# facebookresearch/robust-dynrf

Measured on AMD Instinct MI355X. Metric: training rays/sec (Nvidia Balloon1, configs/Nvidia.txt, static+dynamic TensorVMSplit), higher is better.
Workload: dtype f32; 1 GPU; BASELINE.json configs[1]: Nvidia Balloon1, configs/Nvidia.txt, 4096 rays/iter/GPU, 1xMI355X per rank, static+dynamic TensorVMSplit; one step = 5 dynamic + 5 static forward passes, scene-flow MLP, induced flow/disparity, per-frame depth loss, distortion loss, compositor, factor regularisers, full backward, Adam; config=nvidia, stage=stage0, samples_per_ray=115, global_batch=4096, rays_per_gpu=4096, parallelism=ray-sharded dp1, ranks=1, dead_work=executed (work the reference also computes although nothing consumes it)

## Files before the change

include/rodynrf.h:

```cpp
#ifndef RODYNRF_H
#define RODYNRF_H
#include <stddef.h>
#include <stdint.h>

#ifdef __cplusplus
extern "C" {
#endif

#define RDRF_ABI_VERSION 6

typedef void* rdrf_stream_t;

enum { RDRF_RAY_NDC = 0, RDRF_RAY_CONTRACT = 1, RDRF_RAY_OTHER = 2 };
enum { RDRF_ACT_RELU = 0, RDRF_ACT_SOFTPLUS = 1 };
enum { RDRF_HEAD_MLP_FEA = 0, RDRF_HEAD_MLP_FEA_TIMEEMBEDDING = 1 };
enum { RDRF_SCATTER_RAY = 0, RDRF_SCATTER_SORTED = 1, RDRF_SCATTER_AUTO = 2, RDRF_SCATTER_SORTED_PLAIN = 3 };

typedef struct {
  float* plane[3];
  float* line[3];
  int C[3];
  int H[3], W[3];
  int L[3];
  int sH[3], sW[3];
// ... 321 lines not shown
                      float* y, void* ws, size_t ws_bytes, rdrf_stream_t stream);

#define RDRF_ST_F32 0
#define RDRF_ST_F32_T 1
#define RDRF_ST_B3 2
#define RDRF_ST_B3_T 3
#define RDRF_ST_B3_PAIR_T 4
#define RDRF_ST_B3S 5
#define RDRF_ST_B3S_T 6
int rdrf_selftest_layer(int form, const float* x, const float* w, int M, int K, int OUT, float* y, void* ws, size_t ws_bytes,
                        rdrf_stream_t stream);

#define RDRF_DW_DENSITY 0
#define RDRF_DW_STATIC_FEA 1
#define RDRF_DW_STATIC_TE 2
#define RDRF_DW_DYN_APP 3
#define RDRF_DW_DYN 4
#define RDRF_DW_SCENE_FLOW 5
#define RDRF_DW_FEAT_STATIC 6
#define RDRF_DW_FEAT_DYN 7
#define RDRF_DW_LIVE_D 1
#define RDRF_DW_LIVE_B 2
#define RDRF_DW_SMALL_IN_KERNEL 4
int rdrf_selftest_dw(int plan, int flags, const float* A, size_t A_floats, const float* B, size_t B_floats, int ntiles,
                     const int* count, const void* grads, rdrf_stream_t stream);
int rdrf_selftest_dw_describe(int plan, int flags, int* out, int cap);
int rdrf_selftest_sf_geometry(int ntiles, int* grid, int* waves);

void rdrf_prof_reset(void);
int rdrf_prof_enable(int on);
int rdrf_prof_get(const char* kernel, double* total_ms, int* launches);

#ifdef __cplusplus
}
#endif
#endif
```

robust-dynrf_amd/_lib.py:

```python
import ctypes as C
import os

import torch

_HERE = os.path.dirname(os.path.abspath(__file__))
DETERMINISTIC = os.environ.get("RDRF_DETERMINISTIC", "0") == "1"
LIB_PATH = os.environ.get("RDRF_LIB", os.path.join(_HERE, "librodynrf_det.so" if DETERMINISTIC else "librodynrf.so"))

ABI_VERSION = 6

RAY_TYPES = {"ndc": 0, "contract": 1}
ACTS = {"relu": 0, "softplus": 1}
HEADS = {"MLP_Fea": 0, "MLP_Fea_TimeEmbedding": 1}
SAVE_NO_APP = 1

fp = C.POINTER(C.c_float)


class RdrfVM(C.Structure):
    _fields_ = [("plane", C.c_void_p * 3), ("line", C.c_void_p * 3), ("C", C.c_int * 3),
                ("H", C.c_int * 3), ("W", C.c_int * 3), ("L", C.c_int * 3),
                ("sH", C.c_int * 3), ("sW", C.c_int * 3)]


# ... 102 lines not shown
    lib.rdrf_render_chunks_maps_fwd.argtypes = [C.c_void_p, C.c_void_p, C.c_void_p, C.c_void_p, C.c_void_p, C.c_void_p,
                                                C.c_int, C.c_int, C.c_int, C.c_float, C.c_float, C.POINTER(RenderMapsC),
                                                C.c_void_p, C.c_size_t, C.c_void_p, C.c_void_p, C.c_int]
    lib.rdrf_render_motion_workspace_bytes.restype = C.c_size_t
    lib.rdrf_render_motion_workspace_bytes.argtypes = [C.c_int, C.c_int]
    lib.rdrf_render_motion_fwd.argtypes = [C.c_void_p, C.c_void_p, C.c_void_p, C.c_void_p, C.c_void_p, C.c_void_p, C.c_int,
                                           C.c_int, C.c_float, C.c_float, C.c_int, C.POINTER(RenderMapsC),
                                           C.POINTER(MotionCamsC), C.POINTER(MotionMapsC), C.c_void_p, C.c_size_t, C.c_void_p]
    lib.rdrf_flow_to_image_workspace_bytes.restype = C.c_size_t
    lib.rdrf_flow_to_image_workspace_bytes.argtypes = [C.c_int, C.c_int]
    lib.rdrf_flow_to_image.argtypes = [C.c_void_p, C.c_int, C.c_int, C.c_void_p, C.c_void_p, C.c_size_t, C.c_void_p]
    lib.rdrf_camera_rays.argtypes = [C.c_void_p, C.c_void_p, C.c_int, C.c_int, C.c_int, C.c_int, C.c_float, C.c_int64,
                                     C.c_int, C.c_void_p, C.c_void_p]
    lib.rdrf_ssim_workspace_bytes.restype = C.c_size_t
    lib.rdrf_ssim_workspace_bytes.argtypes = [C.c_int, C.c_int, C.c_int]
    lib.rdrf_ssim.argtypes = [C.c_void_p, C.c_void_p, C.c_int, C.c_int, C.c_int, C.c_float, C.c_void_p, C.c_void_p,
                              C.c_void_p, C.c_size_t, C.c_void_p]
    lib.rdrf_gather_batch.argtypes = [C.POINTER(SceneTablesC), C.c_void_p, C.c_void_p, C.c_int, C.POINTER(BatchC), C.c_void_p]
    lib.rdrf_selftest_layer.argtypes = [C.c_int, C.c_void_p, C.c_void_p, C.c_int, C.c_int, C.c_int, C.c_void_p, C.c_void_p,
                                        C.c_size_t, C.c_void_p]
    lib.rdrf_selftest_dw.argtypes = [C.c_int, C.c_int, C.c_void_p, C.c_size_t, C.c_void_p, C.c_size_t, C.c_int, C.c_void_p,
                                     C.c_void_p, C.c_void_p]
    lib.rdrf_selftest_dw_describe.argtypes = [C.c_int, C.c_int, C.POINTER(C.c_int), C.c_int]
    lib.rdrf_prof_get.argtypes = [C.c_char_p, C.POINTER(C.c_double), C.POINTER(C.c_int)]
    lib.rdrf_det_bind.argtypes = [C.c_int, C.c_void_p, C.c_size_t, C.c_void_p, C.c_void_p]
    lib.rdrf_det_finish.argtypes = [C.c_int, C.c_void_p]
    if DETERMINISTIC and not lib.rdrf_deterministic():
        raise ImportError(f"RDRF_DETERMINISTIC=1 but {LIB_PATH} is the product build")
    return lib


lib = _load()

SYMBOLS = [
    "rdrf_abi_version", "rdrf_last_error", "rdrf_workspace_bytes", "rdrf_forward_workspace_bytes", "rdrf_saved_bytes", "rdrf_saved_bytes_ex", "rdrf_saved_row_bytes",
    "rdrf_generate_rays",
    "rdrf_generate_rays_bwd", "rdrf_generate_rays_uv", "rdrf_generate_rays_uv_bwd", "rdrf_sample_ndc", "rdrf_sample_contract", "rdrf_sample_bwd",
    "rdrf_static_fwd", "rdrf_static_fwd_ex", "rdrf_static_bwd", "rdrf_dynamic_fwd", "rdrf_dynamic_fwd_ex", "rdrf_dynamic_bwd",
    "rdrf_features_saved_bytes", "rdrf_features_workspace_bytes", "rdrf_features_bwd_workspace_bytes",
    "rdrf_static_features_fwd", "rdrf_static_features_bwd", "rdrf_dynamic_features_fwd",
    "rdrf_dynamic_features_bwd",
    "rdrf_scene_flow_fwd", "rdrf_scene_flow_bwd", "rdrf_composite_fwd", "rdrf_composite_bwd",
    "rdrf_induce_flow_fwd", "rdrf_induce_flow_bwd", "rdrf_rows_scatter_add", "rdrf_distloss_fwd", "rdrf_distloss_bwd",
    "rdrf_tv_fwd", "rdrf_tv_bwd", "rdrf_tv_grad", "rdrf_adam_step", "rdrf_upsample_bilinear", "rdrf_dense_l1_fwd",
    "rdrf_dense_l1_bwd", "rdrf_pack_floats", "rdrf_static_pack", "rdrf_dynamic_pack", "rdrf_loss_terms_workspace_floats", "rdrf_loss_terms_fwd", "rdrf_loss_terms_bwd",
    "rdrf_loss_terms_stats", "rdrf_loss_terms_finish", "rdrf_deterministic", "rdrf_det_bind", "rdrf_det_finish",
    "rdrf_render_fused_fwd", "rdrf_render_sequence_fwd",
    "rdrf_frame_depth_loss_workspace_bytes", "rdrf_frame_depth_loss_fwd", "rdrf_frame_depth_loss_bwd",
    "rdrf_render_workspace_bytes", "rdrf_render_fwd", "rdrf_render_chunks_workspace_bytes", "rdrf_render_chunks_fwd",
    "rdrf_render_maps_fwd", "rdrf_render_chunks_maps_fwd", "rdrf_camera_rays", "rdrf_ssim_workspace_bytes", "rdrf_ssim",
    "rdrf_render_motion_workspace_bytes", "rdrf_render_motion_fwd", "rdrf_flow_to_image_workspace_bytes", "rdrf_flow_to_image",
    "rdrf_gather_batch",
    "rdrf_set_scatter_mode", "rdrf_selftest_mlp", "rdrf_selftest_layer", "rdrf_selftest_dw", "rdrf_selftest_dw_describe",
    "rdrf_selftest_sf_geometry",
    "rdrf_prof_reset",
    "rdrf_prof_enable", "rdrf_prof_get",
]


SELFTEST_FORMS = {"F32": 0, "F32_T": 1, "B3": 2, "B3_T": 3, "B3_PAIR_T": 4, "B3S": 5, "B3S_T": 6}

DW_PLANS = {"DENSITY": 0, "STATIC_FEA": 1, "STATIC_TE": 2, "DYN_APP": 3, "DYN": 4, "SCENE_FLOW": 5, "FEAT_STATIC": 6, "FEAT_DYN": 7}
DW_LIVE_D, DW_LIVE_B, DW_SMALL_IN_KERNEL = 1, 2, 4

SCATTER_MODES = {"ray": 0, "sorted": 1, "auto": 2, "sorted_plain": 3}


def set_scatter_mode(mode):
    check(lib.rdrf_set_scatter_mode(SCATTER_MODES[mode]), "rdrf_set_scatter_mode")


class RdrfTensor4(C.Structure):
    _fields_ = [("x", C.c_void_p), ("g", C.c_void_p), ("C", C.c_int), ("H", C.c_int), ("W", C.c_int),
                ("sC", C.c_longlong), ("sH", C.c_longlong), ("sW", C.c_longlong)]


TV_MAX = 16


class RdrfLossTerm(C.Structure):
    _fields_ = [("x", C.c_void_p), ("y", C.c_void_p), ("w", C.c_void_p), ("gx", C.c_void_p), ("gy", C.c_void_p),
                ("rows", C.c_longlong), ("cols", C.c_int), ("kind", C.c_int), ("norm", C.c_int),
                ("ysign", C.c_float), ("coef", C.c_float), ("coef_dev", C.c_void_p)]


MAX_LOSS_TERMS = 32
# ... 66 lines not shown
```

robust-dynrf_amd/csrc/rdrf_bwd.hip:

```cpp
#ifdef RDRF_GROWS_TEMPORAL
#define RDRF_SAVE_TEMPORAL
#endif
#include "rdrf_bwd_dev.hpp"
#include "rdrf_bwd_host.hpp"

RDRF_DET_UNIT(bwd)

RDRF_D void x0_bwd(const float (&X0)[32], const float (&dX0)[32], int h, float& d0, float& d1,
                   float& d2) {
#pragma unroll
  for (int o = 0; o < 8; ++o) {
    if (o == 0 && h == 0) {
      d0 += dX0[0]; d1 += dX0[1]; d2 += dX0[2];
    } else {
      const int k = 2 * o + h - 1;
#pragma unroll
      for (int p = 0; p < 2; ++p) {
        const int j = 2 * k + p;
        const int d = j / 10, f = j - d * 10;
        const float sv = X0[o * 4 + 2 * p], cv = X0[o * 4 + 2 * p + 1];
        const float dq = ldexpf(dX0[o * 4 + 2 * p] * cv - dX0[o * 4 + 2 * p + 1] * sv, f);
        d0 += d == 0 ? dq : 0.f; d1 += d == 1 ? dq : 0.f; d2 += d == 2 ? dq : 0.f;
      }
    }
  }
}

RDRF_D float act_grad(float f, int act, float shift) {
  return act == RDRF_ACT_RELU ? (f > 0.0f ? 1.0f : 0.0f) : sigmoidf_(f + shift);
}

template <int KK, int NO>
// ... 1159 lines not shown
      const int rr = e >> 6, hh = (e >> 5) & 1, c = e & 31;
      const int col = seg_imap(layer == 0 ? SEG_SF_X : SEG_IDENT, 32 * k + c, in_dim);
      const int orow = bo * 32 + (rr & 3) + 8 * (rr >> 2) + 4 * hh;
      if (col >= 0) grad_add(G.w[layer] + (size_t)orow * in_dim + col, red[p * 1024 + e]);
    }
  }
#pragma unroll
  for (int a = 0; a < sfd::NDZ; ++a) {
    const int layer = 2 - (a >> 1), orow = (a & 1) * 32 + (int)threadIdx.x;
    if (threadIdx.x < 32)
      grad_add(G.b[layer] + orow, red[sfd::NPROD * 1024 + a * 64 + threadIdx.x] + red[sfd::NPROD * 1024 + a * 64 + 32 + threadIdx.x]);
  }
  for (int e = threadIdx.x; e < 12 * 32 + 6; e += blockDim.x) {
    const int a = e < 12 * 32 ? e >> 5 : 12 + (e - 12 * 32), c = e < 12 * 32 ? e & 31 : 0;
    const float* r = red + sfd::NPROD * 1024 + (sfd::NDZ + a) * 64 + c;
    if (a < 12) grad_add(G.w[3] + (a >> 1) * 64 + (a & 1) * 32 + c, r[0] + r[32]);
    else grad_add(G.b[3] + (a - 12), r[0] + r[32]);
  }
}
void scene_flow_fused_geometry(long tiles, int* grid, int* waves) {
  const long blocks = (tiles + SFD_WAVES - 1) / SFD_WAVES;
  *grid = (int)(blocks < 1 ? 1 : (blocks > 256 ? 256 : blocks));
  *waves = SFD_WAVES;
}

void fill_static_w(StaticW& w, const RdrfStaticParams* P);
void fill_dyn_w(DynW& w, const RdrfDynamicParams* P);

static void dyn_pack_jobs_bwd(PackJobs& J, const RdrfDynamicParams* P) {
  using namespace pkb;
  J.n = 0;
  const int kh = REG_K1H, kw = REG_K1W, k3 = REG_K3, sf = REG_SF;
  pack_add(J, P->l5w, 64, 3, 64, SEG_IDENT, 1, 3, 32, kw + K1W_W5);
#ifdef RDRF_HEADS_BWD_F32
  const int wm = 2;
#else
  const int wm = 8;
#endif
  pack_add(J, P->l4w, 64, 64, 64, SEG_IDENT, wm, 2, 32, kw + K1W_W4T);
  pack_add(J, P->l3w, 93, 64, 93, SEG_WARP3_X0, wm, 2, 32, kw + K1W_W3T_X0);
  pack_add(J, P->l3w, 93, 64, 93, SEG_WARP3_T, wm, 1, 32, kw + K1W_W3T_T);
  pack_add(J, P->dw2, 64, 1, 64, SEG_IDENT, 1, 1, 32, kh + K1H_DEN2);
  pack_add(J, P->bw2, 64, 1, 64, SEG_IDENT, 1, 1, 32, kh + K1H_BLE2);
#ifdef RDRF_HEADS_BWD_F32
  const int hm = 2;
#else
// ... 97 lines not shown
  b.dxn = dynamic ? c.take<float>(ns * 3) : nullptr;
  b.dtout = dynamic ? c.take<float>((size_t)N * 32) : nullptr;
  b.gf = dynamic ? nullptr : c.take<float>(t1 * 32);
  b.dfs = nullptr;
  b.dfa = nullptr;
  b.gsig = b.dtp = nullptr;
  if (dynamic) {
    b.dfs = c.take<float>(ns * DFS_FLOATS);
    b.dfa = c.take<float>(ns * DFA_FLOATS);
    b.keys_in = c.take<unsigned>(3 * ns);
    b.keys_out = c.take<unsigned>(3 * ns);
    b.order = c.take<unsigned>(3 * ns);
    b.counts = c.take<int>(64);
    b.sort_tmp_bytes = rdrf_sort_temp_bytes((unsigned)(3 * ns), 32);
    b.sort_tmp = c.take<char>(b.sort_tmp_bytes);
    b.gsig = c.take<float>(ns);
    b.dtp = c.take<float>(t3 * 64);
  }
  RDRF_CHECK(c.ok(), -3, "backward workspace too small: need %zu have %zu", c.off, ws_bytes);
  return 0;
}

void add_density_phase_dw(DwJobs& D, const float* grows1, const float* act1, const RdrfDynamicParams* G, int T1, bool live_d,
                          bool live_b, bool small_in_kernel) {
  dw_add(D, grows1, sv::K1G_ROWS, sv::K1G_DZ3, 2, 64, 0, act1, sv::K1_ROWS, 93, 93, G->l3w, G->l3b, nullptr, T1);
  dw_blk(D, sv::K1_X0, SEG_WARP3_X0, 0);
  dw_blk(D, sv::K1_X0 + 32, SEG_WARP3_X0, 32);
  dw_blk(D, sv::K1_T, SEG_WARP3_T, 0);
  dw_add(D, grows1, sv::K1G_ROWS, sv::K1G_DZ4, 2, 64, 0, act1, sv::K1_ROWS, 64, 64, G->l4w, G->l4b, nullptr, T1);
  dw_blk(D, sv::K1_H3, SEG_IDENT, 0);
  dw_blk(D, sv::K1_H3 + 32, SEG_IDENT, 32);
  if (!small_in_kernel) {
  dw_add(D, grows1, sv::K1G_ROWS, sv::K1G_SM, 1, 3, 0, act1, sv::K1_ROWS, 64, 64, G->l5w, G->l5b, nullptr, T1);
  dw_blk(D, sv::K1_H4, SEG_IDENT, 0);
  dw_blk(D, sv::K1_H4 + 32, SEG_IDENT, 32);
  if (live_d) {
    dw_add(D, grows1, sv::K1G_ROWS, sv::K1G_SM, 1, 1, 3, act1, sv::K1_ROWS, 64, 64, G->dw2, G->db2, nullptr, T1);
    dw_blk(D, sv::K1_HD, SEG_IDENT, 0);
    dw_blk(D, sv::K1_HD + 32, SEG_IDENT, 32);
  }
  if (live_b) {
    dw_add(D, grows1, sv::K1G_ROWS, sv::K1G_SM, 1, 1, 4, act1, sv::K1_ROWS, 64, 64, G->bw2, G->bb2, nullptr, T1);
    dw_blk(D, sv::K1_HB, SEG_IDENT, 0);
    dw_blk(D, sv::K1_HB + 32, SEG_IDENT, 32);
  }
  }
  for (int head = 0; head < 2; ++head) {
    if (!(head ? live_b : live_d)) continue;
    dw_add(D, grows1, sv::K1G_ROWS, head ? sv::K1G_DZB : sv::K1G_DZD, 2, 64, 0, act1, sv::K1_ROWS, 152, 152,
           head ? G->bw1 : G->dw1, head ? G->bb1 : G->db1, nullptr, T1);
    const int f0 = head ? sv::K1_FB : sv::K1_FD;
    dw_blk(D, f0, SEG_IDENT72, 0);
    dw_blk(D, f0 + 32, SEG_IDENT72, 32);
    dw_blk(D, f0 + 64, SEG_IDENT72, 64);
    dw_blk(D, sv::K1_X0, SEG_DEN1_X0, 0);
    dw_blk(D, sv::K1_X0 + 32, SEG_DEN1_X0, 32);
    dw_blk(D, sv::K1_X1, SEG_DEN1_X1, 0);
  }
}
void add_static_app_dw(DwJobs& D, const float* grows3, const float* act3, const RdrfStaticParams* G, bool fea, const int* cnt,
                       int ntiles) {
  const int in1 = fea ? 138 : 135;
  dw_add(D, grows3, sv::K3G_ROWS, sv::K3G_DZV, 1, 3, 0, act3, sv::S3_ROWS, 128,
         fea ? 128 : 131, G->w3, G->b3, cnt, ntiles);
  for (int i = 0; i < 4; ++i) dw_blk(D, sv::S3_H2 + 32 * i, SEG_IDENT, 32 * i);
  if (!fea) dw_blk(D, sv::S3_VD, SEG_VIEW3, 0);
  dw_add(D, grows3, sv::K3G_ROWS, sv::K3G_DF, 1, 27, 0, act3, sv::S3_ROWS, 72, 72, G->basis,
         nullptr, cnt, ntiles);
  for (int i = 0; i < 3; ++i) dw_blk(D, sv::S3_G + 32 * i, SEG_IDENT, 32 * i);
  dw_add(D, grows3, sv::K3G_ROWS, sv::K3G_DZ2, 4, 128, 0, act3, sv::S3_ROWS, 128, 128, G->w2,
         G->b2, cnt, ntiles);
  for (int i = 0; i < 4; ++i) dw_blk(D, sv::S3_H1 + 32 * i, SEG_IDENT, 32 * i);
  dw_add(D, grows3, sv::K3G_ROWS, sv::K3G_DZ1, 4, 128, 0, act3, sv::S3_ROWS, in1, in1, G->w1,
         G->b1, cnt, ntiles);
  dw_blk(D, sv::S3_F, fea ? SEG_STAT1_F_FEA : SEG_STAT1_F_TE, 0);
  for (int i = 0; i < 4; ++i) dw_blk(D, sv::S3_P + 32 * i, fea ? SEG_STAT1_P_FEA : SEG_STAT1_P_TE, 32 * i);
}
void add_dyn_app_dw(DwJobs& D, const float* grows3, const float* act3, const RdrfDynamicParams* G, const int* cnt, int ntiles) {
  dw_add(D, grows3, sv::K3G_ROWS, sv::K3G_DZV, 1, 3, 0, act3, sv::K3_ROWS, 128, 131, G->rwv,
         G->rbv, cnt, ntiles);
  for (int i = 0; i < 4; ++i) dw_blk(D, sv::K3_H2 + 32 * i, SEG_IDENT, 32 * i);
// ... 195 lines not shown
    } else RDRF_LAUNCH("dyn_heads_bwd", (k_dyn_density_bwd<0, false>), dim3(g.grid), dim3(g.block), stream, a, w, gw);
    if (smode != 0) {
      const int set_mask = ((g_sigma != nullptr || g_weight != nullptr) ? 1 : 0) | (g_blending != nullptr ? 2 : 0);
      if (set_mask != 0) {
        rdrf_prof_begin("scatter_dyn_density", stream);
        rc = scatter_dyn_density_sorted(a, b, P, G, set_mask, stream);
        rdrf_prof_end("scatter_dyn_density", stream);
        if (rc) return rc;
      }
    } else {
      const bool has_d = g_sigma != nullptr || g_weight != nullptr, has_b = g_blending != nullptr;
      if (has_d || has_b) {
        ScatterArgs sa;
        fill_scatter_common(sa, a);
        sa.nsets = 0;
        if (has_d) { sa.vm[sa.nsets] = P->density; sa.gvm[sa.nsets] = G->density; sa.row0[sa.nsets] = sv::K1G_DFD; ++sa.nsets; }
        if (has_b) { sa.vm[sa.nsets] = P->blending; sa.gvm[sa.nsets] = G->blending; sa.row0[sa.nsets] = sv::K1G_DFB; ++sa.nsets; }
        sa.rows = b.grows1; sa.stride = sv::K1G_ROWS; sa.flat = flat ? 1 : 0;
        sa.xw = a.sp.xw;
        sa.dxw = b.dxw; sa.dxw_accumulate = 1;
        { int rc_ = launch_scatter("scatter_dyn_density", SCATTER_4_1_9, sa, (long)t1, stream); if (rc_) return rc_; }
      }
    }
    if (flat) RDRF_LAUNCH("dyn_warp_bwd", (k_dyn_density_bwd<1, false, true>), dim3(g.grid), dim3(g.block), stream, a, w, gw);
    else RDRF_LAUNCH("dyn_warp_bwd", (k_dyn_density_bwd<1, false>), dim3(g.grid), dim3(g.block), stream, a, w, gw);
    RDRF_LAUNCH("time_branch_bwd", k_time_branch_bwd, dim3((N + TB_RPB - 1) / TB_RPB), dim3(128), stream, ts, w,
                N, b.dtout, flat ? (const float*)b.dtp : nullptr, S, G->l1w, G->l1b, G->l2w, G->l2b);
    const bool small_in_kernel = a.small_dw != 0;
    add_density_phase_dw(D, b.grows1, a.sp.act1, G, (int)t1, g_sigma != nullptr || g_weight != nullptr, g_blending != nullptr,
                         small_in_kernel);
  }
  rc = dw_launch(D, stream, "dw_dyn");
  return rc;
}

struct FeatWs {
  float *pk, *grows3, *grows1, *dxw, *dxn, *dtout, *gpad, *xpad;
  uint8_t* valid;
};
static int carve_feat_bwd(FeatWs& b, void* ws, size_t ws_bytes, int M, int dynamic) {
  WsCarver c(ws, ws_bytes);
  const size_t t = ((size_t)M + 31) / 32, mp = t * 32;
  b.pk = c.take<float>(PACK_AREA_FLOATS);
  b.grows3 = c.take<float>(t * sv::K3G_ROWS * 32);
  b.grows1 = dynamic ? c.take<float>(t * sv::K1G_ROWS * 32) : nullptr;
  b.dxw = dynamic ? c.take<float>(mp * 3) : nullptr;
  b.dxn = dynamic ? c.take<float>(mp * 3) : nullptr;
  b.dtout = dynamic ? c.take<float>(mp * 32) : nullptr;
  b.gpad = dynamic ? nullptr : c.take<float>(mp);
  b.xpad = dynamic ? nullptr : c.take<float>(mp * 3);
  b.valid = c.take<uint8_t>(mp);
  RDRF_CHECK(c.ok(), -3, "features backward: workspace too small: need %zu have %zu", c.off, ws_bytes);
  return 0;
// ... 184 lines not shown
  const int T = (int)tiles;
  DwJobs D;
  D.n = 0;
  add_scene_flow_dw(D, grows, act, G, T);
  return dw_launch(D, stream, "dw_sf");
}

void dyn_pack_jobs_fwd(PackJobs& J, const RdrfDynamicParams* P);
void static_pack_jobs_fwd(PackJobs& J, const RdrfStaticParams* P, int head);
extern "C" size_t rdrf_pack_floats(void) { return PACK_AREA_FLOATS; }
extern "C" int rdrf_static_pack(const RdrfStaticParams* P, int static_head, int backward, float* image,
                                rdrf_stream_t stream_) {
  RDRF_CHECK(P && image && (((uintptr_t)image) & 15) == 0, -1, "static_pack: bad arguments");
  PackJobs J;
  if (backward) static_pack_jobs_bwd(J, P, static_head); else static_pack_jobs_fwd(J, P, static_head);
  return pack_launch(J, image, (hipStream_t)stream_);
}
extern "C" int rdrf_dynamic_pack(const RdrfDynamicParams* P, int backward, float* image, rdrf_stream_t stream_) {
  RDRF_CHECK(P && image && (((uintptr_t)image) & 15) == 0, -1, "dynamic_pack: bad arguments");
  PackJobs J;
  if (backward) dyn_pack_jobs_bwd(J, P); else dyn_pack_jobs_fwd(J, P);
  return pack_launch(J, image, (hipStream_t)stream_);
}
```

robust-dynrf_amd/csrc/rdrf_bwd_host.hpp:

```cpp
#pragma once
#include "rdrf_host.hpp"

struct BwdArgs;

struct BwdWs {
  float* dfs;
  float* dfa;
  unsigned *keys_in, *keys_out, *order;
  int* counts;
  void* sort_tmp;
  size_t sort_tmp_bytes;
  float* pk;
  float* gf;
  float* grows1;
  float* grows3;
  float* dxw;
  float* dxn;
  float* dtout;
  float* gsig;
  float* dtp;
};

struct ScatterArgs {
  RdrfVM vm[2], gvm[2];
// ... 33 lines not shown
  const float* A;
  int A_stride, A_row0, nbo, out_dim, out_row0;
  const float* B;
  int B_stride;
  int nblk;
  int blk_row0[8], blk_seg[8], blk_e0[8];
  int in_dim, ld;
  float* dW;
  float* db;
  const int* count;
  int ntiles;
};
#define RDRF_MAX_DW_JOBS 12
struct DwJobs {
  DwJob j[RDRF_MAX_DW_JOBS];
  int n;
};
void dw_add(DwJobs& D, const float* A, int A_stride, int A_row0, int nbo, int out_dim, int out_row0, const float* B,
            int B_stride, int in_dim, int ld, float* dW, float* db, const int* count, int ntiles);
void dw_blk(DwJobs& D, int row0, int seg, int e0);
int dw_launch(DwJobs& D, hipStream_t stream, const char* name);

void add_density_phase_dw(DwJobs& D, const float* grows1, const float* act1, const RdrfDynamicParams* G, int T1,
                          bool live_d = true, bool live_b = true, bool small_in_kernel = false);
void add_static_app_dw(DwJobs& D, const float* grows3, const float* act3, const RdrfStaticParams* G, bool fea, const int* cnt,
                       int ntiles);
void add_dyn_app_dw(DwJobs& D, const float* grows3, const float* act3, const RdrfDynamicParams* G, const int* cnt, int ntiles);
void add_scene_flow_dw(DwJobs& D, const float* grows, const float* act, const RdrfDynamicParams* G, int T);
void add_feat_static_dw(DwJobs& D, const float* grows3, const float* act3, const RdrfStaticParams* G, int Np);
void add_feat_dyn_app_dw(DwJobs& D, const float* grows3, const float* act3, const RdrfDynamicParams* G, int Np);
void scene_flow_fused_geometry(long tiles, int* grid, int* waves);
```

robust-dynrf_amd/csrc/rdrf_selftest.hip:

```cpp
#include "rdrf_bwd_host.hpp"

namespace {

template <int KK>
RDRF_D void st_load(float (&in)[KK], const float* __restrict__ x, int row, int M, int ld, int c0, int h) {
#pragma unroll
  for (int kk = 0; kk < KK; ++kk) in[kk] = row < M ? x[(size_t)row * ld + c0 + elem_of(kk, h)] : 0.f;
}
template <int NBO>
RDRF_D void st_store(const f32x16 (&acc)[NBO], float* __restrict__ y, int row, int M, int ld, int c0, int h) {
  if (row < M)
#pragma unroll
    for (int nb = 0; nb < NBO; ++nb)
#pragma unroll
      for (int r = 0; r < 16; ++r) y[(size_t)row * ld + c0 + nb * 32 + elem_of(r, h)] = acc[nb][r];
}

template <int NBO, int KK>
__global__ __launch_bounds__(64) void k_st_f32(const float* __restrict__ x, const float* __restrict__ pkw, int M,
                                               float* __restrict__ y) {
  constexpr int IMG = NBO * KK * 64;
  __shared__ __attribute__((aligned(16))) float lds[IMG];
  lds_fill(lds, pkw, IMG);
  const int lane = threadIdx.x & 63, h = lane >> 5, row = blockIdx.x * 32 + (lane & 31);
// ... 169 lines not shown
      if (OUT == 32 && nbi == 3) ST_RUN(img + nbi * kk * 32, (k_st_b3s_t<3, 16>));
      if (OUT == 128 && nbi == 4) ST_RUN(img + nbi * kk * 32, (k_st_b3s_t<4, 64>));
      if (OUT == 128 && nbi == 3) ST_RUN(img + nbi * kk * 32, (k_st_b3s_t<3, 64>));
      if (OUT == 128 && nbi == 5) ST_RUN(img + nbi * kk * 32, (k_st_b3s_t<5, 64>));
      break;
    }
  }
  rdrf_set_error("selftest_layer: form %d is not instantiated for K = %d, OUT = %d", form, K, OUT);
  return -1;
}

namespace {

struct DwPlanInfo {
  int dynamic;
  int region[RDRF_MAX_DW_JOBS];
  int nregions;
};

int dw_plan_jobs(int plan, int flags, const float* A, const float* B, size_t ntiles, const int* count, const void* G, DwJobs& D,
                 DwPlanInfo& I) {
  const RdrfStaticParams* Gs = (const RdrfStaticParams*)G;
  const RdrfDynamicParams* Gd = (const RdrfDynamicParams*)G;
  const bool live_d = (flags & RDRF_DW_LIVE_D) != 0, live_b = (flags & RDRF_DW_LIVE_B) != 0, small = (flags & RDRF_DW_SMALL_IN_KERNEL) != 0;
  const int T = (int)ntiles, Tc = count ? 0 : T;
  D.n = 0;
  I.dynamic = 1;
  int n0 = -1;
  const float *A1 = nullptr, *B1 = nullptr;
  auto second = [&]() {
    n0 = D.n;
    A1 = A + ntiles * (size_t)D.j[0].A_stride * 32;
    B1 = B + ntiles * (size_t)D.j[0].B_stride * 32;
  };
  switch (plan) {
    case RDRF_DW_DENSITY: add_density_phase_dw(D, A, B, Gd, T, live_d, live_b, small); break;
    case RDRF_DW_STATIC_FEA: I.dynamic = 0; add_static_app_dw(D, A, B, Gs, true, count, Tc); break;
    case RDRF_DW_STATIC_TE: I.dynamic = 0; add_static_app_dw(D, A, B, Gs, false, count, Tc); break;
    case RDRF_DW_DYN_APP: add_dyn_app_dw(D, A, B, Gd, count, Tc); break;
    case RDRF_DW_DYN:
      add_dyn_app_dw(D, A, B, Gd, count, Tc);
      second();
      add_density_phase_dw(D, A1, B1, Gd, T, live_d, live_b, small);
      break;
    case RDRF_DW_SCENE_FLOW: add_scene_flow_dw(D, A, B, Gd, T); break;
    case RDRF_DW_FEAT_STATIC: I.dynamic = 0; add_feat_static_dw(D, A, B, Gs, T); break;
    case RDRF_DW_FEAT_DYN:
      add_feat_dyn_app_dw(D, A, B, Gd, T);
      second();
      add_density_phase_dw(D, A1, B1, Gd, T, live_d, live_b);
      break;
    default: rdrf_set_error("selftest_dw: unknown plan %d", plan); return -1;
  }
  I.nregions = n0 < 0 ? 1 : 2;
  for (int j = 0; j < D.n; ++j) I.region[j] = (n0 >= 0 && j >= n0) ? 1 : 0;
  return 0;
}

}

extern "C" int rdrf_selftest_dw(int plan, int flags, const float* A, size_t A_floats, const float* B, size_t B_floats, int ntiles,
                                const int* count, const void* grads, rdrf_stream_t stream_) {
  hipStream_t stream = (hipStream_t)stream_;
  DwJobs D;
  DwPlanInfo I;
  RDRF_CHECK(plan >= RDRF_DW_DENSITY && plan <= RDRF_DW_FEAT_DYN, -1, "selftest_dw: unknown plan %d", plan);
// ... 43 lines not shown
    while (j < D.n && I.region[j] != g) ++j;
    out[n++] = D.j[j].A_stride; out[n++] = D.j[j].B_stride; out[n++] = D.j[j].count != nullptr ? 1 : 0;
  }
  for (int j = 0; j < D.n; ++j) {
    const DwJob& J = D.j[j];
    out[n++] = I.region[j]; out[n++] = J.A_row0; out[n++] = J.nbo; out[n++] = J.out_dim; out[n++] = J.out_row0;
    out[n++] = J.in_dim; out[n++] = J.ld;
    out[n++] = (int)((uintptr_t)J.dW - 8);
    out[n++] = J.db != nullptr ? (int)((uintptr_t)J.db - 8) : -1;
    out[n++] = J.nblk;
    for (int k = 0; k < J.nblk; ++k) {
      out[n++] = J.blk_row0[k];
      for (int li = 0; li < 32; ++li) out[n++] = seg_imap(J.blk_seg[k], J.blk_e0[k] + li, J.in_dim);
    }
  }
  return n;
}

extern "C" int rdrf_selftest_sf_geometry(int ntiles, int* grid, int* waves) {
  RDRF_CHECK(ntiles >= 0 && grid && waves, -1, "selftest_sf_geometry: bad arguments");
  scene_flow_fused_geometry(ntiles, grid, waves);
  return 0;
}
```

Baseline: 460,200 rays/s.

## Fuse warp-MLP backward with its weight-gradient reductions into one kernel

Adds a fused warp-branch backward kernel that computes the layer 3/4/5 activation gradients and also accumulates the weight and bias gradients in registers through MFMA outer products. Partial sums are reduced across waves in LDS and then added to global memory. The kernel is enabled by default on the flat, small-dw path, and the separate dw jobs for l3/l4 are dropped when it runs. The goal is to avoid writing dz3/dz4 rows to global memory and launching dw GEMM jobs for them. The cost is higher register and LDS pressure and a grid capped at 256 blocks, which can limit occupancy.

```diff
diff --git a/include/rodynrf.h b/include/rodynrf.h
--- a/include/rodynrf.h
+++ b/include/rodynrf.h
@@ -367,10 +367,17 @@
 #define RDRF_DW_LIVE_D 1
 #define RDRF_DW_LIVE_B 2
 #define RDRF_DW_SMALL_IN_KERNEL 4
+#define RDRF_DW_WARP_IN_KERNEL 8
 int rdrf_selftest_dw(int plan, int flags, const float* A, size_t A_floats, const float* B, size_t B_floats, int ntiles,
                      const int* count, const void* grads, rdrf_stream_t stream);
 int rdrf_selftest_dw_describe(int plan, int flags, int* out, int cap);
 int rdrf_selftest_sf_geometry(int ntiles, int* grid, int* waves);
+int rdrf_selftest_warp_geometry(int ntiles, int* grid, int* waves);
+size_t rdrf_selftest_warp_bwd_workspace_bytes(int N, int S);
+int rdrf_selftest_warp_bwd(const RdrfDynamicParams* P, const RdrfFieldCfg* cfg, int N, int S, const float* act1,
+                           size_t act1_floats, float* grows1, size_t grows1_floats, float* dxw, float* dxn,
+                           const float* g_xyz_prime, const RdrfDynamicParams* grads, float* g_xyz, float* dtout, float* dtp,
+                           void* ws, size_t ws_bytes, rdrf_stream_t stream);
 
 void rdrf_prof_reset(void);
 int rdrf_prof_enable(int on);
diff --git a/robust-dynrf_amd/_lib.py b/robust-dynrf_amd/_lib.py
--- a/robust-dynrf_amd/_lib.py
+++ b/robust-dynrf_amd/_lib.py
@@ -148,6 +148,12 @@
     lib.rdrf_selftest_dw.argtypes = [C.c_int, C.c_int, C.c_void_p, C.c_size_t, C.c_void_p, C.c_size_t, C.c_int, C.c_void_p,
                                      C.c_void_p, C.c_void_p]
     lib.rdrf_selftest_dw_describe.argtypes = [C.c_int, C.c_int, C.POINTER(C.c_int), C.c_int]
+    lib.rdrf_selftest_warp_geometry.argtypes = [C.c_int, C.POINTER(C.c_int), C.POINTER(C.c_int)]
+    lib.rdrf_selftest_warp_bwd_workspace_bytes.restype = C.c_size_t
+    lib.rdrf_selftest_warp_bwd_workspace_bytes.argtypes = [C.c_int, C.c_int]
+    lib.rdrf_selftest_warp_bwd.argtypes = [C.c_void_p, C.c_void_p, C.c_int, C.c_int, C.c_void_p, C.c_size_t, C.c_void_p, C.c_size_t,
+                                           C.c_void_p, C.c_void_p, C.c_void_p, C.c_void_p, C.c_void_p, C.c_void_p, C.c_void_p,
+                                           C.c_void_p, C.c_size_t, C.c_void_p]
     lib.rdrf_prof_get.argtypes = [C.c_char_p, C.POINTER(C.c_double), C.POINTER(C.c_int)]
     lib.rdrf_det_bind.argtypes = [C.c_int, C.c_void_p, C.c_size_t, C.c_void_p, C.c_void_p]
     lib.rdrf_det_finish.argtypes = [C.c_int, C.c_void_p]
@@ -178,7 +184,7 @@
     "rdrf_render_motion_workspace_bytes", "rdrf_render_motion_fwd", "rdrf_flow_to_image_workspace_bytes", "rdrf_flow_to_image",
     "rdrf_gather_batch",
     "rdrf_set_scatter_mode", "rdrf_selftest_mlp", "rdrf_selftest_layer", "rdrf_selftest_dw", "rdrf_selftest_dw_describe",
-    "rdrf_selftest_sf_geometry",
+    "rdrf_selftest_sf_geometry", "rdrf_selftest_warp_geometry", "rdrf_selftest_warp_bwd_workspace_bytes", "rdrf_selftest_warp_bwd",
     "rdrf_prof_reset",
     "rdrf_prof_enable", "rdrf_prof_get",
 ]
@@ -187,7 +193,7 @@
 SELFTEST_FORMS = {"F32": 0, "F32_T": 1, "B3": 2, "B3_T": 3, "B3_PAIR_T": 4, "B3S": 5, "B3S_T": 6}
 
 DW_PLANS = {"DENSITY": 0, "STATIC_FEA": 1, "STATIC_TE": 2, "DYN_APP": 3, "DYN": 4, "SCENE_FLOW": 5, "FEAT_STATIC": 6, "FEAT_DYN": 7}
-DW_LIVE_D, DW_LIVE_B, DW_SMALL_IN_KERNEL = 1, 2, 4
+DW_LIVE_D, DW_LIVE_B, DW_SMALL_IN_KERNEL, DW_WARP_IN_KERNEL = 1, 2, 4, 8
 
 SCATTER_MODES = {"ray": 0, "sorted": 1, "auto": 2, "sorted_plain": 3}
 
diff --git a/robust-dynrf_amd/csrc/rdrf_bwd.hip b/robust-dynrf_amd/csrc/rdrf_bwd.hip
--- a/robust-dynrf_amd/csrc/rdrf_bwd.hip
+++ b/robust-dynrf_amd/csrc/rdrf_bwd.hip
@@ -8,6 +8,7 @@
 
 RDRF_D void x0_bwd(const float (&X0)[32], const float (&dX0)[32], int h, float& d0, float& d1,
                    float& d2) {
+#pragma clang fp contract(off)
 #pragma unroll
   for (int o = 0; o < 8; ++o) {
     if (o == 0 && h == 0) {
@@ -1213,6 +1214,264 @@
   const long blocks = (tiles + SFD_WAVES - 1) / SFD_WAVES;
   *grid = (int)(blocks < 1 ? 1 : (blocks > 256 ? 256 : blocks));
   *waves = SFD_WAVES;
+}
+
+namespace wpd {
+constexpr int WAVES = SFD_WAVES;
+constexpr int ST_SIZE = 64 * 32;
+constexpr int NPROD = 10, NDZ = 4, NSM = 6;
+constexpr int LDS = pkb::K1W_SIZE + WAVES * ST_SIZE;
+constexpr int RED = NPROD * 1024 + (NDZ + NSM) * 64;
+static_assert(pkb::K1W_SIZE % 4 == 0 && RED <= LDS && LDS * 4 <= 160 * 1024, "the cross-wave sum reuses the kernel's LDS");
+}
+struct WarpGrads {
+  float *l3w, *l3b, *l4w, *l4b;
+};
+RDRF_D void x0_bwd_flat(const float (&X0)[32], const float (&dX0)[32], int h, float& d0, float& d1, float& d2) {
+#pragma clang fp contract(off)
+  d0 += h == 0 ? dX0[0] : 0.f; d1 += h == 0 ? dX0[1] : 0.f; d2 += h == 0 ? dX0[2] : 0.f;
+#pragma unroll
+  for (int o = 0; o < 8; ++o) {
+    const int k = 2 * o + h - 1;
+#pragma unroll
+    for (int p = 0; p < 2; ++p) {
+      const int j = 2 * k + p;
+      const int d = j >= 0 ? j / 10 : -1, f = j >= 0 ? j - d * 10 : 0;
+      const float sv = X0[o * 4 + 2 * p], cv = X0[o * 4 + 2 * p + 1];
+      const float dq = ldexpf(dX0[o * 4 + 2 * p] * cv - dX0[o * 4 + 2 * p + 1] * sv, f);
+      d0 += d == 0 ? dq : 0.f; d1 += d == 1 ? dq : 0.f; d2 += d == 2 ? dq : 0.f;
+    }
+  }
+}
+
+template <bool GX>
+__global__ __launch_bounds__(64 * wpd::WAVES) void k_dyn_warp_bwd_dw(BwdArgs a, DynG gw, WarpGrads G) {
+  __shared__ __attribute__((aligned(16))) float lds[wpd::LDS];
+  const int lane = threadIdx.x & 63, h = lane >> 5, s = lane & 31;
+  const int wave = __builtin_amdgcn_readfirstlane(threadIdx.x >> 6), nwaves = blockDim.x >> 6;
+  float* st = lds + pkb::K1W_SIZE + wave * wpd::ST_SIZE;
+  lds_fill(lds, a.pk + pkb::REG_K1W, pkb::K1W_SIZE);
+  const int total = a.N * a.S;
+  const int ntiles = (total + 31) >> 5;
+  const SfdPos pos = sfd_lane_pos(s, h);
+  f32x16 accW[wpd::NPROD];
+  float bsum[wpd::NDZ];
+  float sw[3] = {0.f, 0.f, 0.f}, sb[3] = {0.f, 0.f, 0.f};
+  acc_zero<wpd::NPROD>(accW);
+#pragma unroll
+  for (int i = 0; i < wpd::NDZ; ++i) bsum[i] = 0.f;
+  for (int n = blockIdx.x * nwaves + wave; n < ntiles; n += gridDim.x * nwaves) {
+    const bool act = n * 32 + s < total;
+    const int idx = act ? n * 32 + s : 0;
+    const float* svb = a.sp.act1 + (size_t)n * sv::K1_ROWS * 32;
+    float* gb = a.grows1 + (size_t)n * sv::K1G_ROWS * 32;
+    float dw0 = act ? a.dxw_app[(size_t)idx * 3 + 0] : 0.f, dw1 = act ? a.dxw_app[(size_t)idx * 3 + 1] : 0.f,
+          dw2 = act ? a.dxw_app[(size_t)idx * 3 + 2] : 0.f;
+    float dn0 = act ? a.dxn_app[(size_t)idx * 3 + 0] : 0.f, dn1 = act ? a.dxn_app[(size_t)idx * 3 + 1] : 0.f,
+          dn2 = act ? a.dxn_app[(size_t)idx * 3 + 2] : 0.f;
+    float dd0 = dw0 * a.box.inv[0], dd1 = dw1 * a.box.inv[1], dd2 = dw2 * a.box.inv[2];
+    float gp0 = 0.f, gp1 = 0.f, gp2 = 0.f;
+    if (act && a.g_xyz_prime) {
+      gp0 = a.g_xyz_prime[(size_t)idx * 3 + 0]; gp1 = a.g_xyz_prime[(size_t)idx * 3 + 1];
+      gp2 = a.g_xyz_prime[(size_t)idx * 3 + 2];
+    }
+    dd0 += gp0; dd1 += gp1; dd2 += gp2;
+    if (!act) { dd0 = dd1 = dd2 = 0.f; }
+    if (h == 0) {
+      gb[(size_t)(sv::K1G_SM + 0) * 32 + s] = dd0; gb[(size_t)(sv::K1G_SM + 1) * 32 + s] = dd1;
+      gb[(size_t)(sv::K1G_SM + 2) * 32 + s] = dd2;
+    }
+    float dz4[32];
+    {
+      float H4[32];
+      load_rows<32>(svb, sv::K1_H4, H4, s, h);
+      const float* w5 = lds + pkb::K1W_W5 + h * 32;
+#pragma unroll
+      for (int q = 0; q < 8; ++q) {
+        const f32x4 wa = *reinterpret_cast<const f32x4*>(w5 + 4 * q);
+        const f32x4 wb = *reinterpret_cast<const f32x4*>(w5 + 64 + 4 * q);
+        const f32x4 wc = *reinterpret_cast<const f32x4*>(w5 + 128 + 4 * q);
+#pragma unroll
+        for (int c = 0; c < 4; ++c) {
+          const float d = wa[c] * dd0 + wb[c] * dd1 + wc[c] * dd2;
+          dz4[4 * q + c] = H4[4 * q + c] > 0.f ? d : 0.f;
+        }
+      }
+      sb[0] += dd0; sb[1] += dd1; sb[2] += dd2;
+#pragma unroll 1
+      for (int o = 0; o < 3; ++o) {
+        const float dd = o == 0 ? dd0 : (o == 1 ? dd1 : dd2);
+        float pw[32];
+#pragma unroll
+        for (int kk = 0; kk < 32; ++kk) pw[kk] = dd * H4[kk];
+        const float r = reduce_scatter32(pw, s);
+        sw[0] += o == 0 ? r : 0.f; sw[1] += o == 1 ? r : 0.f; sw[2] += o == 2 ? r : 0.f;
+      }
+    }
+    f32x4 b0[4], b1[4], b2[4];
+    sfd_wave_sync();
+    sfd_stage(st, dz4, pos);
+    sfd_wave_sync();
+    sfd_load(b0, svb, sv::K1_H3 + s, h);
+    sfd_load(b1, svb, sv::K1_H3 + 32 + s, h);
+    float dz3[32];
+    {
+      f32x16 acc[2];
+      acc_zero<2>(acc);
+#ifdef RDRF_HEADS_BWD_F32
+      mfma_seg<2, 32>(acc, dz4, lds + pkb::K1W_W4T, lane);
+#else
+      mfma_seg_b3<2, 32>(acc, dz4, lds + pkb::K1W_W4T, lane);
+#endif
+      float H3[32];
+      load_rows<32>(svb, sv::K1_H3, H3, s, h);
+#pragma unroll
+      for (int bo = 0; bo < 2; ++bo) {
+        f32x4 av[4];
+        sfd_read(av, st, bo, pos);
+        bsum[bo] += sfd_sum(av);
+        sfd_prod(accW[2 * bo], av, b0);
+        sfd_prod(accW[2 * bo + 1], av, b1);
+        __builtin_amdgcn_sched_barrier(0);
+      }
+#pragma unroll
+      for (int kk = 0; kk < 32; ++kk) dz3[kk] = H3[kk] > 0.f ? acc[kk >> 4][kk & 15] : 0.f;
+    }
+    sfd_wave_sync();
+    sfd_stage(st, dz3, pos);
+    sfd_wave_sync();
+    sfd_load(b0, svb, sv::K1_X0 + s, h);
+    sfd_load(b1, svb, sv::K1_X0 + 32 + s, h);
+    sfd_load(b2, svb, sv::K1_T + s, h);
+    f32x16 accX[2];
+    {
+      float dXh[32];
+      load_rows<32>(gb, sv::K1G_DX0, dXh, s, h);
+#pragma unroll
+      for (int kk = 0; kk < 32; ++kk) accX[kk >> 4][kk & 15] = dXh[kk];
+    }
+    f32x16 accT[1];
+    acc_zero<1>(accT);
+#ifdef RDRF_HEADS_BWD_F32
+    mfma_seg<2, 32>(accX, dz3, lds + pkb::K1W_W3T_X0, lane);
+    mfma_seg<1, 32>(accT, dz3, lds + pkb::K1W_W3T_T, lane);
+#else
+    mfma_seg_b3_pair<2, 1, 32>(accX, accT, dz3, lds + pkb::K1W_W3T_X0, lds + pkb::K1W_W3T_T, lane);
+#endif
+#pragma unroll
+    for (int bo = 0; bo < 2; ++bo) {
+      f32x4 av[4];
+      sfd_read(av, st, bo, pos);
+      bsum[2 + bo] += sfd_sum(av);
+      sfd_prod(accW[4 + 3 * bo], av, b0);
+      sfd_prod(accW[4 + 3 * bo + 1], av, b1);
+      sfd_prod(accW[4 + 3 * bo + 2], av, b2);
+      __builtin_amdgcn_sched_barrier(0);
+    }
+    {
+      float X0[32], dX0[32];
+      load_rows<32>(svb, sv::K1_X0, X0, s, h);
+      acc_copy<2>(dX0, accX);
+      float e0 = 0.f, e1 = 0.f, e2 = 0.f;
+      x0_bwd_flat(X0, dX0, h, e0, e1, e2);
+      e0 += __shfl_xor(e0, 32, 64); e1 += __shfl_xor(e1, 32, 64); e2 += __shfl_xor(e2, 32, 64);
+      dn0 += e0 + dw0; dn1 += e1 + dw1; dn2 += e2 + dw2;
+    }
+    if constexpr (GX) {
+      const __amdgpu_buffer_rsrc_t rp = __builtin_amdgcn_make_buffer_rsrc((void*)(a.g_xyz + (size_t)n * 96), 0, 384, 0x00020000);
+      const int off = (act && h == 0) ? s * 12 : 1 << 20;
+      const float p0 = __builtin_bit_cast(float, __builtin_amdgcn_raw_buffer_load_b32(rp, off, 0, 0));
+      const float p1 = __builtin_bit_cast(float, __builtin_amdgcn_raw_buffer_load_b32(rp, off, 4, 0));
+      const float p2 = __builtin_bit_cast(float, __builtin_amdgcn_raw_buffer_load_b32(rp, off, 8, 0));
+      __builtin_amdgcn_raw_buffer_store_b32(__builtin_bit_cast(unsigned, p0 + (dn0 * a.box.inv[0] + gp0)), rp, off, 0, 0);
+      __builtin_amdgcn_raw_buffer_store_b32(__builtin_bit_cast(unsigned, p1 + (dn1 * a.box.inv[1] + gp1)), rp, off, 4, 0);
+      __builtin_amdgcn_raw_buffer_store_b32(__builtin_bit_cast(unsigned, p2 + (dn2 * a.box.inv[2] + gp2)), rp, off, 8, 0);
+    }
+    {
+      const int i0 = n * 32 + s, nl = i0 / a.S, nl0 = (n * 32) / a.S;
+      const int rb = nl * a.S - n * 32, re = rb + a.S - 1;
+      const int end = re < 31 ? re : 31;
+      const bool head = i0 < total && (s == 0 || rb == s);
+      const bool inside = rb >= 0 && re <= 31;
+      const int nrays = a.N - nl0 < 32 ? a.N - nl0 : 32;
+      const __amdgpu_buffer_rsrc_t rt = __builtin_amdgcn_make_buffer_rsrc((void*)(a.dtout + (size_t)nl0 * 32), 0, nrays * 128, 0x00020000);
+      const __amdgpu_buffer_rsrc_t rq = __builtin_amdgcn_make_buffer_rsrc((void*)(a.dtp + (size_t)n * 64), 0, 256, 0x00020000);
+      const int offt = (head && inside) ? (nl - nl0) * 128 + h * 16 : 1 << 20;
+      const int offq = (head && !inside) ? (s == 0 ? 0 : 128) + h * 16 : 1 << 20;
+#pragma unroll
+      for (int i = 0; i < 16; ++i) {
+        float v = 0.f + accT[0][i];
+#pragma unroll
+        for (int d = 1; d < 32; d <<= 1) {
+          const float o = __shfl_down(v, d, 32);
+          v += s + d <= end ? o : 0.f;
+        }
+        const int eo = (8 * (i >> 2) + (i & 3)) * 4;
+        __builtin_amdgcn_raw_buffer_store_b32(__builtin_bit_cast(unsigned, v), rt, offt, eo, 0);
+        __builtin_amdgcn_raw_buffer_store_b32(__builtin_bit_cast(unsigned, v), rq, offq, eo, 0);
+      }
+    }
+  }
+  float sm[wpd::NSM];
+#pragma unroll
+  for (int o = 0; o < 3; ++o) {
+    sm[o] = sw[o];
+    sm[3 + o] = wave_sum(h == 0 ? sb[o] : 0.f);
+  }
+  float* red = lds;
+  for (int w = 0; w < nwaves; ++w) {
+    __syncthreads();
+    if (wave == w) {
+#pragma unroll
+      for (int p = 0; p < wpd::NPROD; ++p)
+#pragma unroll
+        for (int rr = 0; rr < 16; ++rr) {
+          float* r = red + p * 1024 + rr * 64 + lane;
+          *r = w == 0 ? accW[p][rr] : *r + accW[p][rr];
+        }
+#pragma unroll
+      for (int i = 0; i < wpd::NDZ; ++i) {
+        float* r = red + wpd::NPROD * 1024 + i * 64 + lane;
+        *r = w == 0 ? bsum[i] : *r + bsum[i];
+      }
+#pragma unroll
+      for (int i = 0; i < wpd::NSM; ++i) {
+        float* r = red + wpd::NPROD * 1024 + (wpd::NDZ + i) * 64 + lane;
+        *r = w == 0 ? sm[i] : *r + sm[i];
+      }
+    }
+  }
+  __syncthreads();
+#pragma unroll
+  for (int p = 0; p < wpd::NPROD; ++p) {
+    const bool l4 = p < 4;
+    const int bo = l4 ? p >> 1 : (p - 4) / 3, k = l4 ? p & 1 : (p - 4) % 3;
+    const int ld = l4 ? 64 : 93;
+    float* dW = l4 ? G.l4w : G.l3w;
+    for (int e = threadIdx.x; e < 1024; e += blockDim.x) {
+      const int rr = e >> 6, hh = (e >> 5) & 1, c = e & 31;
+      const int col = l4 ? 32 * k + c : (k < 2 ? seg_imap(SEG_WARP3_X0, 32 * k + c, 93) : seg_imap(SEG_WARP3_T, c, 93));
+      const int orow = bo * 32 + (rr & 3) + 8 * (rr >> 2) + 4 * hh;
+      if (col >= 0) grad_add(dW + (size_t)orow * ld + col, red[p * 1024 + e]);
+    }
+  }
+#pragma unroll
+  for (int i = 0; i < wpd::NDZ; ++i) {
+    float* db = i < 2 ? G.l4b : G.l3b;
+    const int orow = (i & 1) * 32 + (int)threadIdx.x;
+    if (threadIdx.x < 32)
+      grad_add(db + orow, red[wpd::NPROD * 1024 + i * 64 + threadIdx.x] + red[wpd::NPROD * 1024 + i * 64 + 32 + threadIdx.x]);
+  }
+  for (int e = threadIdx.x; e < 3 * 64 + 3; e += blockDim.x) {
+    const float* r = red + wpd::NPROD * 1024 + wpd::NDZ * 64;
+    if (e < 192) grad_add(gw.l5w + (e >> 6) * 64 + elem_of(e & 31, (e >> 5) & 1), r[e]);
+    else grad_add(gw.l5b + (e - 192), r[(3 + e - 192) * 64]);
+  }
+}
+void warp_fused_geometry(long tiles, int* grid, int* waves) {
+  const long blocks = (tiles + wpd::WAVES - 1) / wpd::WAVES;
+  *grid = (int)(blocks < 1 ? 1 : (blocks > 256 ? 256 : blocks));
+  *waves = wpd::WAVES;
 }
 
 void fill_static_w(StaticW& w, const RdrfStaticParams* P);
@@ -1356,7 +1615,8 @@
 }
 
 void add_density_phase_dw(DwJobs& D, const float* grows1, const float* act1, const RdrfDynamicParams* G, int T1, bool live_d,
-                          bool live_b, bool small_in_kernel) {
+                          bool live_b, bool small_in_kernel, bool warp_in_kernel) {
+  if (!warp_in_kernel) {
   dw_add(D, grows1, sv::K1G_ROWS, sv::K1G_DZ3, 2, 64, 0, act1, sv::K1_ROWS, 93, 93, G->l3w, G->l3b, nullptr, T1);
   dw_blk(D, sv::K1_X0, SEG_WARP3_X0, 0);
   dw_blk(D, sv::K1_X0 + 32, SEG_WARP3_X0, 32);
@@ -1364,6 +1624,7 @@
   dw_add(D, grows1, sv::K1G_ROWS, sv::K1G_DZ4, 2, 64, 0, act1, sv::K1_ROWS, 64, 64, G->l4w, G->l4b, nullptr, T1);
   dw_blk(D, sv::K1_H3, SEG_IDENT, 0);
   dw_blk(D, sv::K1_H3 + 32, SEG_IDENT, 32);
+  }
   if (!small_in_kernel) {
   dw_add(D, grows1, sv::K1G_ROWS, sv::K1G_SM, 1, 3, 0, act1, sv::K1_ROWS, 64, 64, G->l5w, G->l5b, nullptr, T1);
   dw_blk(D, sv::K1_H4, SEG_IDENT, 0);
@@ -1391,6 +1652,19 @@
     dw_blk(D, sv::K1_X0 + 32, SEG_DEN1_X0, 32);
     dw_blk(D, sv::K1_X1, SEG_DEN1_X1, 0);
   }
+}
+static bool warp_fused_path(bool flat, bool small_dw) {
+  static const int fused = RDRF_ENV("RDRF_WARP_FUSED") ? atoi(RDRF_ENV("RDRF_WARP_FUSED")) : 1;
+  return flat && small_dw && fused != 0;
+}
+static int launch_warp_fused(const BwdArgs& a, const DynG& gw, const RdrfDynamicParams* G, long tiles, hipStream_t stream) {
+  int grid, waves;
+  warp_fused_geometry(tiles, &grid, &waves);
+  WarpGrads wg;
+  wg.l3w = G->l3w; wg.l3b = G->l3b; wg.l4w = G->l4w; wg.l4b = G->l4b;
+  if (a.g_xyz != nullptr) RDRF_LAUNCH("dyn_warp_bwd", k_dyn_warp_bwd_dw<true>, dim3(grid), dim3(64 * waves), stream, a, gw, wg);
+  else RDRF_LAUNCH("dyn_warp_bwd", k_dyn_warp_bwd_dw<false>, dim3(grid), dim3(64 * waves), stream, a, gw, wg);
+  return 0;
 }
 void add_static_app_dw(DwJobs& D, const float* grows3, const float* act3, const RdrfStaticParams* G, bool fea, const int* cnt,
                        int ntiles) {
@@ -1632,13 +1906,15 @@
         { int rc_ = launch_scatter("scatter_dyn_density", SCATTER_4_1_9, sa, (long)t1, stream); if (rc_) return rc_; }
       }
     }
-    if (flat) RDRF_LAUNCH("dyn_warp_bwd", (k_dyn_density_bwd<1, false, true>), dim3(g.grid), dim3(g.block), stream, a, w, gw);
+    const bool warp_fused = warp_fused_path(flat, a.small_dw != 0);
+    if (warp_fused) { int rc_ = launch_warp_fused(a, gw, G, (long)t1, stream); if (rc_) return rc_; }
+    else if (flat) RDRF_LAUNCH("dyn_warp_bwd", (k_dyn_density_bwd<1, false, true>), dim3(g.grid), dim3(g.block), stream, a, w, gw);
     else RDRF_LAUNCH("dyn_warp_bwd", (k_dyn_density_bwd<1, false>), dim3(g.grid), dim3(g.block), stream, a, w, gw);
     RDRF_LAUNCH("time_branch_bwd", k_time_branch_bwd, dim3((N + TB_RPB - 1) / TB_RPB), dim3(128), stream, ts, w,
                 N, b.dtout, flat ? (const float*)b.dtp : nullptr, S, G->l1w, G->l1b, G->l2w, G->l2b);
     const bool small_in_kernel = a.small_dw != 0;
     add_density_phase_dw(D, b.grows1, a.sp.act1, G, (int)t1, g_sigma != nullptr || g_weight != nullptr, g_blending != nullptr,
-                         small_in_kernel);
+                         small_in_kernel, warp_fused);
   }
   rc = dw_launch(D, stream, "dw_dyn");
   return rc;
@@ -1869,3 +2145,36 @@
   if (backward) dyn_pack_jobs_bwd(J, P); else dyn_pack_jobs_fwd(J, P);
   return pack_launch(J, image, (hipStream_t)stream_);
 }
+
+size_t warp_bwd_on_rows_pack_floats() { return PACK_AREA_FLOATS; }
+int warp_bwd_on_rows(const RdrfDynamicParams* P, const RdrfFieldCfg* cfg, int N, int S, const float* act1, float* grows1,
+                     float* dxw, float* dxn, const float* g_xyz_prime, const RdrfDynamicParams* G, float* g_xyz, float* dtout,
+                     float* dtp, float* pk, uint8_t* valid, hipStream_t stream) {
+  BwdArgs a;
+  fill_bwd_common(a, cfg, nullptr, nullptr, nullptr, nullptr, valid, N, S);
+  a.g_xyz_prime = g_xyz_prime; a.g_xyz = g_xyz;
+  a.small_dw = 1;
+  a.sp.act1 = const_cast<float*>(act1);
+  a.pk = pk; a.grows1 = grows1; a.dxw_app = dxw; a.dxn_app = dxn; a.dtout = dtout; a.dtp = dtp;
+  DynW w;
+  fill_dyn_w(w, P);
+  DynG gw;
+  memset(&gw, 0, sizeof(gw));
+  gw.l5b = G->l5b; gw.l5w = G->l5w;
+  if (P->packed_bwd != nullptr) a.pk = P->packed_bwd;
+  else {
+    PackJobs J;
+    dyn_pack_jobs_bwd(J, P);
+    int rc = pack_launch(J, pk, stream);
+    if (rc) return rc;
+  }
+  const size_t ns = (size_t)N * S, t1 = (ns + 31) / 32;
+  RDRF_FILL(valid, 1, ns, stream);
+  if (warp_fused_path(true, true)) return launch_warp_fused(a, gw, G, (long)t1, stream);
+  const Geo g = geo_for_units((long)t1);
+  RDRF_LAUNCH("dyn_warp_bwd", (k_dyn_density_bwd<1, false, true>), dim3(g.grid), dim3(g.block), stream, a, w, gw);
+  DwJobs D;
+  D.n = 0;
+  add_density_phase_dw(D, grows1, act1, G, (int)t1, false, false, true, false);
+  return dw_launch(D, stream, "dw_warp");
+}
diff --git a/robust-dynrf_amd/csrc/rdrf_bwd_host.hpp b/robust-dynrf_amd/csrc/rdrf_bwd_host.hpp
--- a/robust-dynrf_amd/csrc/rdrf_bwd_host.hpp
+++ b/robust-dynrf_amd/csrc/rdrf_bwd_host.hpp
@@ -79,7 +79,7 @@
 int dw_launch(DwJobs& D, hipStream_t stream, const char* name);
 
 void add_density_phase_dw(DwJobs& D, const float* grows1, const float* act1, const RdrfDynamicParams* G, int T1,
-                          bool live_d = true, bool live_b = true, bool small_in_kernel = false);
+                          bool live_d = true, bool live_b = true, bool small_in_kernel = false, bool warp_in_kernel = false);
 void add_static_app_dw(DwJobs& D, const float* grows3, const float* act3, const RdrfStaticParams* G, bool fea, const int* cnt,
                        int ntiles);
 void add_dyn_app_dw(DwJobs& D, const float* grows3, const float* act3, const RdrfDynamicParams* G, const int* cnt, int ntiles);
@@ -87,3 +87,8 @@
 void add_feat_static_dw(DwJobs& D, const float* grows3, const float* act3, const RdrfStaticParams* G, int Np);
 void add_feat_dyn_app_dw(DwJobs& D, const float* grows3, const float* act3, const RdrfDynamicParams* G, int Np);
 void scene_flow_fused_geometry(long tiles, int* grid, int* waves);
+void warp_fused_geometry(long tiles, int* grid, int* waves);
+int warp_bwd_on_rows(const RdrfDynamicParams* P, const RdrfFieldCfg* cfg, int N, int S, const float* act1, float* grows1,
+                     float* dxw, float* dxn, const float* g_xyz_prime, const RdrfDynamicParams* G, float* g_xyz, float* dtout,
+                     float* dtp, float* pk, uint8_t* valid, hipStream_t stream);
+size_t warp_bwd_on_rows_pack_floats();
diff --git a/robust-dynrf_amd/csrc/rdrf_selftest.hip b/robust-dynrf_amd/csrc/rdrf_selftest.hip
--- a/robust-dynrf_amd/csrc/rdrf_selftest.hip
+++ b/robust-dynrf_amd/csrc/rdrf_selftest.hip
@@ -1,3 +1,4 @@
+#include "rdrf_kernels.hpp"
 #include "rdrf_bwd_host.hpp"
 
 namespace {
@@ -215,7 +216,8 @@
                  DwPlanInfo& I) {
   const RdrfStaticParams* Gs = (const RdrfStaticParams*)G;
   const RdrfDynamicParams* Gd = (const RdrfDynamicParams*)G;
-  const bool live_d = (flags & RDRF_DW_LIVE_D) != 0, live_b = (flags & RDRF_DW_LIVE_B) != 0, small = (flags & RDRF_DW_SMALL_IN_KERNEL) != 0;
+  const bool live_d = (flags & RDRF_DW_LIVE_D) != 0, live_b = (flags & RDRF_DW_LIVE_B) != 0, small = (flags & RDRF_DW_SMALL_IN_KERNEL) != 0,
+             warp = (flags & RDRF_DW_WARP_IN_KERNEL) != 0;
   const int T = (int)ntiles, Tc = count ? 0 : T;
   D.n = 0;
   I.dynamic = 1;
@@ -227,14 +229,14 @@
     B1 = B + ntiles * (size_t)D.j[0].B_stride * 32;
   };
   switch (plan) {
-    case RDRF_DW_DENSITY: add_density_phase_dw(D, A, B, Gd, T, live_d, live_b, small); break;
+    case RDRF_DW_DENSITY: add_density_phase_dw(D, A, B, Gd, T, live_d, live_b, small, warp); break;
     case RDRF_DW_STATIC_FEA: I.dynamic = 0; add_static_app_dw(D, A, B, Gs, true, count, Tc); break;
     case RDRF_DW_STATIC_TE: I.dynamic = 0; add_static_app_dw(D, A, B, Gs, false, count, Tc); break;
     case RDRF_DW_DYN_APP: add_dyn_app_dw(D, A, B, Gd, count, Tc); break;
     case RDRF_DW_DYN:
       add_dyn_app_dw(D, A, B, Gd, count, Tc);
       second();
-      add_density_phase_dw(D, A1, B1, Gd, T, live_d, live_b, small);
+      add_density_phase_dw(D, A1, B1, Gd, T, live_d, live_b, small, warp);
       break;
     case RDRF_DW_SCENE_FLOW: add_scene_flow_dw(D, A, B, Gd, T); break;
     case RDRF_DW_FEAT_STATIC: I.dynamic = 0; add_feat_static_dw(D, A, B, Gs, T); break;
@@ -324,3 +326,32 @@
   scene_flow_fused_geometry(ntiles, grid, waves);
   return 0;
 }
+
+extern "C" int rdrf_selftest_warp_geometry(int ntiles, int* grid, int* waves) {
+  RDRF_CHECK(ntiles >= 0 && grid && waves, -1, "selftest_warp_geometry: bad arguments");
+  warp_fused_geometry(ntiles, grid, waves);
+  return 0;
+}
+
+extern "C" size_t rdrf_selftest_warp_bwd_workspace_bytes(int N, int S) {
+  return warp_bwd_on_rows_pack_floats() * 4 + (((size_t)N * S + 255) & ~(size_t)255) + 512;
+}
+extern "C" int rdrf_selftest_warp_bwd(const RdrfDynamicParams* P, const RdrfFieldCfg* cfg, int N, int S, const float* act1,
+                                      size_t act1_floats, float* grows1, size_t grows1_floats, float* dxw, float* dxn,
+                                      const float* g_xyz_prime, const RdrfDynamicParams* grads, float* g_xyz, float* dtout,
+                                      float* dtp, void* ws, size_t ws_bytes, rdrf_stream_t stream_) {
+  hipStream_t stream = (hipStream_t)stream_;
+  if (N == 0) return 0;
+  RDRF_CHECK(P && cfg && grads && act1 && grows1 && dxw && dxn && dtout && dtp && ws && N > 0 && S > 0 && S <= 4096, -1,
+             "selftest_warp_bwd: bad arguments");
+  RDRF_CHECK((size_t)N * S * 3 < (size_t)INT32_MAX, -1, "selftest_warp_bwd: N * S * 3 must stay below 2^31");
+  RDRF_CHECK((((uintptr_t)act1 | (uintptr_t)grows1 | (uintptr_t)ws) & 15) == 0, -1, "selftest_warp_bwd: rows and workspace must be 16-byte aligned");
+  const size_t tiles = ((size_t)N * S + 31) / 32;
+  RDRF_CHECK(act1_floats >= tiles * sv::K1_ROWS * 32 && grows1_floats >= tiles * sv::K1G_ROWS * 32, -3,
+             "selftest_warp_bwd: rows too small for %zu tiles", tiles);
+  RDRF_CHECK(ws_bytes >= rdrf_selftest_warp_bwd_workspace_bytes(N, S), -3, "selftest_warp_bwd: workspace too small");
+  WsCarver c(ws, ws_bytes);
+  float* pk = c.take<float>(warp_bwd_on_rows_pack_floats());
+  uint8_t* valid = c.take<uint8_t>((size_t)N * S);
+  return warp_bwd_on_rows(P, cfg, N, S, act1, grows1, dxw, dxn, g_xyz_prime, grads, g_xyz, dtout, dtp, pk, valid, stream);
+}
```

Result: faster. 469,200 rays/s, median of 6 (+2.0%).
